# deepmarkpy/aware

Hardware: AMD Instinct MI355X
Metric: waveform-seconds/sec through embed->attack->detect; BER vs reference (higher is better)
Workload: dtype f32 accumulation on the 16-bit MFMA pipe; conv-block GEMMs: every f32 operand scaled by a power of two and carried as TWO binary16 terms (within one f32 ulp of the operand, rms 2^-24.5), 3 partial products, the l_a*l_b term (<= 2^-22) dropped -- gemm_h2.hip: error level of an f32 dot product (agains

## Files before the change

aware_amd/csrc/capi.hip:

```cpp
#include <hip/hip_runtime.h>
#include <math.h>
#include <stdio.h>
#include <stdlib.h>
#include <string.h>
#include <string>
#include <algorithm>
#include <vector>

#include "../../include/aware_hip.h"
#include "common.hpp"
#include "kernels.h"

using namespace aware;

static thread_local std::string g_last_err;

#define HIPCHK(expr)                                                                  \
    do {                                                                              \
        hipError_t _e = (expr);                                                       \
        if (_e != hipSuccess) {                                                       \
            g_last_err = std::string(#expr) + ": " + hipGetErrorString(_e);           \
            return AWARE_E_HIP;                                                       \
        }                                                                             \
    } while (0)
#define LAUNCHCHK() HIPCHK(hipGetLastError())

struct LaunchProfiler {
    hipStream_t st;
    std::vector<hipEvent_t> ev;
    std::vector<int> kind;
};
static thread_local LaunchProfiler* g_prof = nullptr;
static inline void prof_mark(int kind) {
    if (!g_prof) return;
    hipEvent_t e;
    if (hipEventCreate(&e) != hipSuccess) return;
    (void)hipEventRecord(e, g_prof->st);
    g_prof->ev.push_back(e);
    g_prof->kind.push_back(kind);
}
#define PROF(kind) prof_mark(kind)
enum { K_SYNTH = 0, K_ANALYSIS = 1, K_GEMM = 2, K_MELNORM = 3, K_INLRELU = 4, K_HEAD = 5, K_SYNTH_ADJ = 6,
       K_ANALYSIS_ADJ = 7, K_MISC = 8, K_GEMM_CLIP_FWD = 9, K_GEMM_CLIP_BWD = 10, K_GEMM_X3_FWD = 11, K_GEMM_X3_BWD = 12 };

static int absmax_into_scratch(const float* in, const int* off, const int* len, int B, int max_len, void* scratch,
                               unsigned long long** pmax_out, int** pcount_out, int* ps_out, hipStream_t st);

struct aware_plan {
    PlanDev dev;
    void* mem = nullptr;
};

struct aware_batch {
    int B = 0;
    std::vector<int> n, in_off, T, frame_off, pool_off, out_off, out_len, pc_in, pc_syn;
    int NF = 0, NP = 0, NS = 0, max_frames = 0, max_len = 0, pstride = 0;
    int uniform_tp = 0;
    int synth_run = kSynthBlocks;
    int* d_mem = nullptr;
    int *d_frame_off = nullptr, *d_pool_off = nullptr, *d_in_off = nullptr, *d_in_len = nullptr, *d_out_off = nullptr,
        *d_out_len = nullptr, *d_pc_in = nullptr, *d_pc_syn = nullptr;
    int an_run = 0, n_an_wg = 0, n_syn_wg = 0;
    int *d_an_wg = nullptr, *d_syn_wg = nullptr;
    std::vector<int> an_wg, syn_wg;
    int* d_order = nullptr;
    std::vector<int> order;
};

struct aware_detector {
    int n_mels = 0, n_layers = 0, nbits = 0;
    int band_lo = 0, nband = 0;
    int ch[8] = {0};
    int maxc = 0;
    float* mem = nullptr;
    float* melT = nullptr;
    float* melB = nullptr;
    float* w[8] = {nullptr};
    float* wT[8] = {nullptr};
    void* wpk[8] = {nullptr};
    void* wTpk[8] = {nullptr};
    void* melTpk = nullptr;
    void* melBpk = nullptr;
    void* lastpk = nullptr;
    void* lastTpk = nullptr;
    void* pkmem = nullptr;
    void* wh2[8] = {nullptr};
    void* wTh2[8] = {nullptr};
    void* h2mem = nullptr;
    float* bias[8] = {nullptr};
    void* mel2mem = nullptr;
    float2* melw = nullptr;
    unsigned char* melm = nullptr;
    float* melf_w = nullptr;
    unsigned char* melf_s = nullptr;
};

extern "C" int aware_version(void) { return 300; }
extern "C" const char* aware_last_hip_error(void) { return g_last_err.c_str(); }

extern "C" int aware_plan_create(aware_plan** out, int n_fft, int hop, int win_length, int window, int band_lo_bin,
                                 int band_hi_bin) {
    if (!out) return AWARE_E_BADARG;
    if (n_fft != kNfft || hop != kHop || win_length != kNfft) return AWARE_E_UNSUPPORTED;
    if (window != 0 && window != 1) return AWARE_E_BADARG;
    const int nband = band_hi_bin - band_lo_bin + 1;
    if (band_lo_bin < 1 || band_hi_bin > 511 || nband < 1 || nband > kFS) return AWARE_E_UNSUPPORTED;
    const double PI = 3.14159265358979323846;
    std::vector<float> h(2 * 512 + 2 * 512 + 1024 + 1024 + 3 * 768);
    float* tw512 = h.data();
    float* tw1024 = tw512 + 1024;
    float* win = tw1024 + 1024;
    float* win2 = win + 1024;
    for (int j = 0; j < 512; ++j) {
        tw512[2 * j] = (float)cos(2 * PI * j / 512);
        tw512[2 * j + 1] = (float)-sin(2 * PI * j / 512);
        tw1024[2 * j] = (float)cos(2 * PI * j / 1024);
        tw1024[2 * j + 1] = (float)-sin(2 * PI * j / 1024);
// ... 41 lines not shown
    b->B = B;
    b->n.assign(n_samples, n_samples + B);
    b->in_off.resize(B);
    b->T.resize(B);
    b->frame_off.resize(B + 1);
    b->pool_off.resize(B + 1);
    b->out_off.resize(B);
    b->out_len.resize(B);
    b->pc_in.resize(B);
    b->pc_syn.resize(B);
    int acc = 0, max_pc = 1;
    for (int rb : {12, 8, 6, 4}) {
        long runs = 0;
        for (int i = 0; i < B; ++i) runs += (n_samples[i] / kHop + rb - 1) / rb;
        bool ok = true;
        for (int i = 0; i < B && ok; ++i) {
            const int nb = n_samples[i] / kHop, ns = (nb + rb - 1) / rb;
            if (ns > 1 && nb / ns < 3) ok = false;
        }
        if (!ok) continue;
        b->synth_run = rb;
        if (runs >= 4096) break;
    }
    b->frame_off[0] = 0;
    b->pool_off[0] = 0;
    for (int i = 0; i < B; ++i) {
        const int n = n_samples[i];
        if (n <= kHalf) { delete b; return AWARE_E_BADARG; }
        b->in_off[i] = in_offsets ? in_offsets[i] : acc;
        acc += n;
        const int T = 1 + n / kHop;
        b->T[i] = T;
        b->frame_off[i + 1] = b->frame_off[i] + T;
        b->pool_off[i + 1] = b->pool_off[i] + ((T / 2 + 31) & ~31);
        b->out_off[i] = kHop * (b->frame_off[i] - i);
        b->out_len[i] = kHop * (T - 1);
        b->pc_in[i] = (n + 4095) / 4096;
        int nseg = (T - 1 + b->synth_run - 1) / b->synth_run;
        if (nseg < 1) nseg = 1;
        b->pc_syn[i] = nseg;
        if (T > b->max_frames) b->max_frames = T;
        if (n > b->max_len) b->max_len = n;
        if (b->pc_in[i] > max_pc) max_pc = b->pc_in[i];
        if (nseg > max_pc) max_pc = nseg;
    }
    b->NF = b->frame_off[B];
    b->NP = b->pool_off[B];
    b->uniform_tp = b->T[0] / 2;
    for (int i = 1; i < B; ++i)
        if (b->T[i] / 2 != b->uniform_tp) b->uniform_tp = 0;
    b->NS = kHop * (b->NF - B);
    b->pstride = max_pc;
    {
        constexpr int kAnalysisMaxRun = 12;
        auto total_runs = [&](int r) { long t = 0; for (int i = 0; i < B; ++i) t += (b->T[i] + r - 1) / r; return t; };
        int R = 4;
        for (int cand = kAnalysisMaxRun; cand >= 4; --cand)
            if (total_runs(cand) >= 4096) { R = cand; break; }
        bool same = true;
        for (int i = 1; i < B; ++i) same = same && b->T[i] == b->T[0];
        if (same)
            for (int cand = R; cand >= 4 && cand >= R - 3; --cand)
                if (((b->T[0] + cand - 1) / cand) % kStreamWaves == 0) { R = cand; break; }
        b->an_run = R;
        if (B < (1 << 19) && b->max_frames / 4 < 4096 * kStreamWaves) {
            for (int i = 0; i < B; ++i) {
                const int ra = (b->T[i] + R - 1) / R, rs = std::max(1, (b->T[i] - 1 + b->synth_run - 1) / b->synth_run);
                for (int w = 0; w < (ra + kStreamWaves - 1) / kStreamWaves; ++w) b->an_wg.push_back((i << 12) | w);
                for (int w = 0; w < (rs + kStreamWaves - 1) / kStreamWaves; ++w) b->syn_wg.push_back((i << 12) | w);
            }
        }
        b->n_an_wg = (int)b->an_wg.size();
        b->n_syn_wg = (int)b->syn_wg.size();
    }
    b->order.resize(B);
    for (int i = 0; i < B; ++i) b->order[i] = i;
    std::stable_sort(b->order.begin(), b->order.end(), [&](int x, int y) { return b->T[x] > b->T[y]; });
    const size_t ints = (size_t)(B + 1) * 2 + (size_t)B * 7 + b->an_wg.size() + b->syn_wg.size();
    HIPCHK(hipMalloc((void**)&b->d_mem, ints * sizeof(int)));
    int* d = b->d_mem;
    auto up = [&](int*& dst, const std::vector<int>& v) -> hipError_t {
        dst = d;
        d += v.size();
        return hipMemcpy(dst, v.data(), v.size() * sizeof(int), hipMemcpyHostToDevice);
    };
    HIPCHK(up(b->d_frame_off, b->frame_off));
    HIPCHK(up(b->d_pool_off, b->pool_off));
    HIPCHK(up(b->d_in_off, b->in_off));
    HIPCHK(up(b->d_in_len, b->n));
    HIPCHK(up(b->d_out_off, b->out_off));
    HIPCHK(up(b->d_out_len, b->out_len));
    HIPCHK(up(b->d_pc_in, b->pc_in));
    HIPCHK(up(b->d_pc_syn, b->pc_syn));
    HIPCHK(up(b->d_order, b->order));
    if (b->n_an_wg) HIPCHK(up(b->d_an_wg, b->an_wg));
    if (b->n_syn_wg) HIPCHK(up(b->d_syn_wg, b->syn_wg));
    *out = b;
    return AWARE_OK;
}
extern "C" void aware_batch_destroy(aware_batch* b) {
    if (!b) return;
    if (b->d_mem) (void)hipFree(b->d_mem);
    delete b;
}
extern "C" int aware_batch_total_frames(const aware_batch* b) { return b ? b->NF : AWARE_E_BADARG; }
extern "C" int aware_batch_total_pooled(const aware_batch* b) { return b ? b->NP : AWARE_E_BADARG; }
extern "C" int aware_batch_total_out(const aware_batch* b) { return b ? b->NS : AWARE_E_BADARG; }
extern "C" int aware_batch_out_offset(const aware_batch* b, int i) {
    return (b && i >= 0 && i < b->B) ? b->out_off[i] : AWARE_E_BADARG;
}
extern "C" int aware_batch_out_length(const aware_batch* b, int i) {
    return (b && i >= 0 && i < b->B) ? b->out_len[i] : AWARE_E_BADARG;
}
extern "C" int aware_batch_frames(const aware_batch* b, int i) {
    return (b && i >= 0 && i < b->B) ? b->T[i] : AWARE_E_BADARG;
}
extern "C" size_t aware_batch_scratch_bytes(const aware_batch* b) {
    return b ? (size_t)b->B * b->pstride * sizeof(unsigned long long) + 256 : 0;
}

static void run_analysis(AnalysisLaunch& L, int dsp_path, hipStream_t st) {
    if (dsp_path == 0 && !L.full && stream_supported(L.plan)) { L.stream = 1; launch_analysis_stream(L, st); }
    else launch_analysis(L, st);
}
static void run_synth(SynthLaunch& S, int dsp_path, hipStream_t st) {
    if (dsp_path == 0 && !S.full && stream_supported(S.plan)) { S.stream = 1; launch_synth_stream(S, st); }
    else launch_synth(S, st);
}

struct Carver {
    char* base;
    size_t off = 0, cap;
    bool ok = true;
    Carver(void* p, size_t c) : base((char*)p), cap(c) {}
    template <typename Tp> Tp* take(size_t count) {
        off = (off + 255) & ~(size_t)255;
        Tp* r = (Tp*)(base + off);
        off += count * sizeof(Tp);
        if (off > cap) ok = false;
        return r;
    }
};

extern "C" int aware_stft(const aware_plan* plan, const aware_batch* b, const float* audio, int normalize, void* spec,
                          void* scratch, void* stream) {
    if (!plan || !b || !audio || !spec || (normalize && !scratch)) return AWARE_E_BADARG;
    hipStream_t st = (hipStream_t)stream;
    unsigned long long* pmax = (unsigned long long*)scratch;
// ... 986 lines not shown
    HIPCHK(hipMemcpyAsync(e->target, target, (size_t)b->B * e->det->nbits * sizeof(float), hipMemcpyDeviceToDevice, st));
    HIPCHK(hipMemsetAsync(e->step, 0, 4 * sizeof(int), st));
    HIPCHK(hipMemsetD32Async((hipDeviceptr_t)e->best_loss, 0x7F800000, b->B, st));
    if (e->opt.active) {
        HIPCHK(hipMemcpyAsync(e->opt.d_lr, e->opt.lr_init.data(), (size_t)b->B * sizeof(double), hipMemcpyHostToDevice, st));
        HIPCHK(hipMemcpyAsync(e->opt.d_state, e->opt.state_init.data(), (size_t)b->B * 3 * sizeof(double), hipMemcpyHostToDevice, st));
    }
    e->steps_done = 0;
    return AWARE_OK;
}

static int embed_iteration(aware_embed* e, hipStream_t st, int do_step, float* grad_out) {
    const aware_batch* b = e->b;
    const aware_detector* d = e->det;
    SynthLaunch S;
    S.plan = e->plan->dev; S.frame_off = b->d_frame_off; S.B = b->B; S.max_frames = b->max_frames; S.run_blocks = b->synth_run; S.wg_tab = b->d_syn_wg; S.n_wg = b->n_syn_wg;
    S.amp = e->coef; S.ph = e->P; S.out = e->yraw; S.add = e->oob; S.pmax = e->pmaxY; S.pstride = b->pstride;
    S.c0 = e->pl1 ? e->c0 : nullptr; S.pl1 = e->pl1;
    const int dsp = e->cfg.dsp_path;
    run_synth(S, dsp, st);
    LAUNCHCHK(); PROF(K_SYNTH);
    if (e->pl1) {
        launch_l1_reduce(e->pl1, b->d_pc_syn, b->pstride, b->d_frame_off, e->plan->dev.nband, e->cfg.l1_weight, e->l1term, b->B, st);
        LAUNCHCHK(); PROF(K_MISC);
    }
    AnalysisLaunch L;
    L.plan = e->plan->dev; L.frame_off = b->d_frame_off; L.B = b->B; L.max_frames = b->max_frames; L.run_frames = b->an_run; L.wg_tab = b->d_an_wg; L.n_wg = b->n_an_wg;
    L.sig = e->yraw; L.sig_off = b->d_out_off; L.sig_len = b->d_out_len;
    L.pmax = e->pmaxY; L.pcount = b->d_pc_syn; L.pstride = b->pstride; L.double_norm = 1;
    L.mag = e->mag; L.unit = e->U; L.unit_default = 0.f; L.write_pad = 0;
    const bool mel_taps = dsp == 0 && d->melw && d->melm && stream_supported(e->plan->dev) && e->cfg.mel == 0;
    const bool mel_fold = mel_taps && d->melf_w && d->melf_s && d->n_mels == 128;
    if (mel_fold) { L.mel_out = e->db.xm; L.melf_w = d->melf_w; L.melf_s = d->melf_s; }
    run_analysis(L, dsp, st);
    LAUNCHCHK(); PROF(K_ANALYSIS);
    DetGradCtx G;
    G.pipe = e->cfg.conv_pipe; G.readout = e->cfg.readout; G.target = e->target; G.loss_kind = e->cfg.loss;
    G.loss = e->loss; G.d1 = e->d1; G.d2 = e->d2; G.gmag = e->gmag; G.loss_add = e->l1term;
    G.step = do_step ? e->step : nullptr;
    G.best_loss = do_step ? e->best_loss : nullptr;
    G.improved = do_step ? e->improved : nullptr;
    G.mel_grad_only = mel_taps;
    G.xm_ready = mel_fold;
    int rc = det_forward_backward(d, b, e->mag, e->db, G, st);
    if (rc) return rc;
    SynthLaunch SA;
    SA.plan = e->plan->dev; SA.frame_off = b->d_frame_off; SA.B = b->B; SA.max_frames = b->max_frames; SA.run_blocks = b->synth_run; SA.wg_tab = b->d_syn_wg; SA.n_wg = b->n_syn_wg;
    SA.amp = e->gmag; SA.ph = e->U; SA.out = e->gy; SA.adjoint = 1; SA.yraw = e->yraw; SA.pmax_in = e->pmaxY;
    SA.pcount = b->d_pc_syn; SA.pdot = e->pdot; SA.pstride = b->pstride; SA.gpad = e->gpad;
    if (mel_taps) { SA.dmel = e->db.xm; SA.melw = d->melw; SA.melm = d->melm; }
    run_synth(SA, dsp, st);
    LAUNCHCHK(); PROF(K_SYNTH_ADJ);
    AnalysisLaunch LA;
    LA.plan = e->plan->dev; LA.frame_off = b->d_frame_off; LA.B = b->B; LA.max_frames = b->max_frames; LA.run_frames = b->an_run; LA.wg_tab = b->d_an_wg; LA.n_wg = b->n_an_wg;
    LA.sig = e->gy; LA.sig_off = b->d_out_off; LA.sig_len = b->d_out_len;
    LA.pmax = e->pmaxY; LA.pcount = b->d_pc_syn; LA.pstride = b->pstride;
    LA.adjoint = 1; LA.yraw = e->yraw; LA.pdot = e->pdot; LA.phasor = e->P;
    LA.coef = e->coef; LA.mom = e->mom; LA.vel = e->vel; LA.lo = e->lo; LA.hi = e->hi; LA.best = e->best;
    LA.improved = e->improved; LA.sched = e->sched; LA.sched_len = e->cfg.num_iterations + 1; LA.step = e->step;
    const bool own_step = do_step && e->opt.active;
    LA.grad_out = own_step ? e->gmag : grad_out; LA.do_step = own_step ? 0 : do_step;
    memcpy(LA.hyp, e->hyp, sizeof(LA.hyp));
    LA.gpad = e->gpad; LA.c0 = e->c0; LA.box_ratio = (float)pow(10.0, -(double)e->cfg.tolerance_db / 20.0);
    LA.l1_weight = e->pl1 ? e->cfg.l1_weight : 0.f;
    run_analysis(LA, dsp, st);
    LAUNCHCHK(); PROF(K_ANALYSIS_ADJ);
    if (own_step) {
        const auto& o = e->opt;
        launch_opt_rows(o.kind, e->coef, e->gmag, e->mom, e->vel, e->c0, LA.box_ratio, e->best, e->improved, b->d_frame_off, b->B,
                        b->NF, o.d_tab, e->cfg.num_iterations, e->step, o.plateau ? o.d_lr : nullptr, o.wd, o.hyp,
                        e->plan->dev.nband, st);
        if (o.plateau)
            launch_plateau(e->loss, o.d_state, o.d_lr, b->B, o.factor, o.patience, o.threshold, o.min_lr, o.eps, st);
        LAUNCHCHK(); PROF(K_MISC);
    }
    return AWARE_OK;
}

extern "C" int aware_embed_iterate(aware_embed* e, int n_iters, void* stream) {
    if (!e || n_iters < 0) return AWARE_E_BADARG;
    if (e->steps_done + n_iters > e->cfg.num_iterations) return AWARE_E_BADARG;
    hipStream_t st = (hipStream_t)stream;
    if (!e->cfg.use_graph) {
        for (int i = 0; i < n_iters; ++i) {
            int rc = embed_iteration(e, st, 1, nullptr);
            if (rc) return rc;
            ++e->steps_done;
        }
        return AWARE_OK;
    }
    constexpr int kGraphIters = 16;
    if (!e->gexec) {
        if (!e->cap) HIPCHK(hipStreamCreateWithFlags(&e->cap, hipStreamNonBlocking));
        for (int which = 0; which < 2; ++which) {
            HIPCHK(hipStreamBeginCapture(e->cap, hipStreamCaptureModeThreadLocal));
            int rc = AWARE_OK;
            for (int i = 0; i < (which ? kGraphIters : 1) && rc == AWARE_OK; ++i) rc = embed_iteration(e, e->cap, 1, nullptr);
            hipGraph_t g = nullptr;
            hipError_t ce = hipStreamEndCapture(e->cap, &g);
            hipGraphExec_t ge = nullptr;
            if (rc == AWARE_OK && ce == hipSuccess) ce = hipGraphInstantiate(&ge, g, nullptr, nullptr, 0);
            if (rc != AWARE_OK || ce != hipSuccess) {
                if (ge) (void)hipGraphExecDestroy(ge);
                if (g) (void)hipGraphDestroy(g);
                if (e->gexec) { (void)hipGraphExecDestroy(e->gexec); e->gexec = nullptr; }
                if (e->graph) { (void)hipGraphDestroy(e->graph); e->graph = nullptr; }
                if (rc != AWARE_OK) return rc;
// ... 254 lines not shown
```

aware_amd/csrc/dsp_stream.hip:

```cpp
#include "common.hpp"
#include "dsp_args.hpp"
#include "kernels.h"

namespace aware {

constexpr int kSW = kStreamWaves;
constexpr int kSThreads = 64 * kSW;

__device__ __forceinline__ ClipNorm clip_norm_wave(const unsigned long long* part, int nseg, int lane) {
    unsigned long long v = 0;
    for (int i = lane; i < nseg; i += 64) v = umax64(v, part[i]);
    v = wave_max64(v);
    ClipNorm c;
    const float raw = __uint_as_float((unsigned)(v >> 32));
    c.k = 0xFFFFFFFFu - (unsigned)(v & 0xFFFFFFFFu);
    c.m = raw + 1e-8f;
    c.m2 = raw / c.m + 1e-8f;
    return c;
}
__device__ __forceinline__ double dot_wave(const double* part, int nseg, int lane) {
    double s = 0.0;
    for (int i = lane; i < nseg; i += 64) s += part[i];
    return wave_sum_d(s);
}

struct LaneEnv {
    float2 lo, hi;
};
__device__ __forceinline__ LaneEnv lane_env(const PlanDev& pl, int lane) {
    LaneEnv e;
    e.lo = make_float2(fast_rcp(pl.env_tab[768 + 2 * lane]), fast_rcp(pl.env_tab[768 + 2 * lane + 1]));
    e.hi = make_float2(fast_rcp(pl.env_tab[768 + 128 + 2 * lane]), fast_rcp(pl.env_tab[768 + 128 + 2 * lane + 1]));
    return e;
}
__device__ __forceinline__ float env_at(const PlanDev& pl, int p, int T) {
    return T < 4 ? ola_envelope_loop(pl.window2, p, T) : pl.env_tab[ola_envelope_index(p, T)];
}

template <int MODE, bool L1, bool MELF = false>
__global__ __launch_bounds__(kSThreads, MODE == AN_ADJ ? 3 : 4) void analysis_stream_kernel(AnalysisArgs a, int run_frames) {
    __shared__ float magrow_s[MELF ? kSW : 1][MELF ? kFS : 1];
    __shared__ cf tw1s[512];
    __shared__ cf tw2s[64];
    __shared__ float2 wins[512];
    __shared__ cf scratch[kSW][kFftScratch];
    const int tid = threadIdx.x;
    fft_fill_tables(tid, kSThreads, a.plan.tw512, tw1s, tw2s);
    for (int i = tid; i < 512; i += kSThreads) wins[i] = make_float2(a.plan.window[2 * i], a.plan.window[2 * i + 1]);
    __syncthreads();

    int b = blockIdx.y, wgx = blockIdx.x;
    if (a.wg_tab) { const int e = a.wg_tab[blockIdx.x]; b = e >> 12; wgx = e & 4095; }
    const int f0 = a.frame_off[b];
    const int T = a.frame_off[b + 1] - f0;
    const int wave = __builtin_amdgcn_readfirstlane(tid >> 6), lane = tid & 63;
    const int t0 = (wgx * kSW + wave) * run_frames;
    if (t0 >= T) return;
    const int nfr = min(run_frames, T - t0);
    const int n = a.sig_len[b];
    const float* x = a.sig + a.sig_off[b];
    const bool al8 = (reinterpret_cast<uintptr_t>(x) & 7) == 0;

    float m = 1.f, m2 = 1.f;
    unsigned kmax = 0xFFFFFFFFu;
    if (a.pmax) {
        const ClipNorm cn = clip_norm_wave(a.pmax + (size_t)b * a.pstride, a.pcount[b], lane);
        m = cn.m;
        m2 = (MODE == AN_ADJ || a.double_norm) ? cn.m2 : 1.f;
        kmax = cn.k;
    }
    const float inv_m = 1.0f / m, inv_m2 = 1.0f / m2, inv_mm2 = 1.0f / (m * m2);
    float corr = 0.f;
    const float* gpL = nullptr;
    const float* gpR = nullptr;
    LaneEnv le;
    le.lo = le.hi = make_float2(1.f, 1.f);
    if (MODE == AN_ADJ) {
        const float adot = (float)dot_wave(a.pdot + (size_t)b * a.pstride, a.pcount[b], lane);
        const float yk = a.yraw[a.sig_off[b] + kmax];
        corr = adot * ((yk > 0.f) ? 1.f : ((yk < 0.f) ? -1.f : 0.f));
        gpL = a.gpad + (size_t)b * 1024;
        gpR = gpL + 512;
        le = lane_env(a.plan, lane);
    }

    auto load_half = [&](int P) -> float2 {
        const int s_lo = P - kHalf;
        float2 v;
        if (MODE == AN_NORM) {
            if (al8 && s_lo >= 0 && s_lo + 128 <= n) {
                v = *reinterpret_cast<const float2*>(x + s_lo + 2 * lane);
            } else {
                int s0 = s_lo + 2 * lane, s1 = s0 + 1;
                s0 = s0 < 0 ? -s0 : s0;
                s1 = s1 < 0 ? -s1 : s1;
                s0 = s0 >= n ? 2 * (n - 1) - s0 : s0;
                s1 = s1 >= n ? 2 * (n - 1) - s1 : s1;
                v.x = x[min(max(s0, 0), n - 1)];
                v.y = x[min(max(s1, 0), n - 1)];
            }
            if (a.pmax) {
                v.x = v.x * inv_m;
                v.y = v.y * inv_m;
                if (a.double_norm) { v.x = v.x * inv_m2; v.y = v.y * inv_m2; }
            }
            return v;
        }
        if (al8 && T >= 4 && s_lo >= 513 && s_lo + 127 <= n - 514 && P >= 768 && P + 127 < kHop * T) {
            float2 g = *reinterpret_cast<const float2*>(x + s_lo + 2 * lane);
            const unsigned s = (unsigned)(s_lo + 2 * lane);
            if (s == kmax) g.x -= corr;
            if (s + 1 == kmax) g.y -= corr;
            g.x = g.x * inv_mm2;
            g.y = g.y * inv_mm2;
            const float2 re = (P & 128) ? le.hi : le.lo;
            return make_float2(g.x * re.x, g.y * re.y);
        }
        float o[2];
#pragma unroll
        for (int e = 0; e < 2; ++e) {
            const int p = P + 2 * lane + e;
            const int src = p - kHalf;
            const bool valid = src >= 0 && src < n;
            float g = x[min(max(src, 0), n - 1)];
            const bool cl = src >= 1 && src <= kHalf;
            const bool cr = src >= n - kHalf - 1 && src <= n - 2;
            const float pl = gpL[min(max(kHalf - src, 0), 511)];
            const float pr = gpR[min(max(n - 2 - src, 0), 511)];
            if (cl) g += pl;
            if (cr) g += pr;
            if ((unsigned)src == kmax) g -= corr;
            g = g * inv_mm2;
            o[e] = valid ? g * fast_rcp(env_at(a.plan, p, T)) : 0.f;
        }
        return make_float2(o[0], o[1]);
    };

    cf* s = scratch[wave];
    const int band_lo = a.plan.band_lo, nband = a.plan.nband;
    cf w1024[5];
#pragma unroll
    for (int r = 0; r < 5; ++r) w1024[r] = a.plan.tw1024[lane + 64 * r];
    float4 sc = make_float4(0.f, 0.f, 1.f, 0.f);
    float inv_bc2 = 1.f;
    int improved = 0;
    if (MODE == AN_ADJ && a.do_step) {
        sc = a.sched[min(max(*a.step - 1, 0), a.sched_len - 1)];
        inv_bc2 = 1.0f / sc.z;
        improved = a.improved[b];
    }

    const float l1g = (MODE == AN_ADJ && L1) ? a.l1_weight / (float)(nband * T) : 0.f;
    float wA[kMelTapsA], wB[kMelTapsB];
    int sA = 0, sB = 0;
    if (MELF) {
#pragma unroll
        for (int j = 0; j < kMelTapsA; ++j) wA[j] = a.melf_w[(size_t)lane * kMelTapsB + j];
#pragma unroll
        for (int j = 0; j < kMelTapsB; ++j) wB[j] = a.melf_w[(size_t)(lane + 64) * kMelTapsB + j];
        sA = a.melf_s[lane];
        sB = a.melf_s[lane + 64];
#pragma unroll
        for (int r = 0; r < 8; ++r) {
            const int f = lane + 64 * r - band_lo;
            if (f >= nband && f < kFS) magrow_s[MELF ? wave : 0][f] = 0.f;
        }
    }
    float2 raw[8];
#pragma unroll
    for (int r = 0; r < 8; ++r) raw[r] = load_half(kHop * t0 + 128 * r);

#pragma unroll 1
    for (int fr = 0; fr < nfr; ++fr) {
        const int t = t0 + fr;
        const size_t row = (size_t)(f0 + t);
        cf preP[5];
        float preM[5], preV[5], preC[5], pre0[5];
        if (MODE == AN_ADJ) {
#pragma unroll
            for (int r = 0; r < 5; ++r) {
                const int f = lane + 64 * r - band_lo;
                const size_t idx = row * kFS + (size_t)min(max(f, 0), kFS - 1);
                preP[r] = a.phasor[idx];
                if (a.do_step) { preM[r] = a.mom[idx]; preV[r] = a.vel[idx]; preC[r] = a.coef[idx]; }
                else { preM[r] = preV[r] = 0.f; preC[r] = L1 ? a.coef[idx] : 0.f; }
                pre0[r] = (a.do_step || L1) ? a.c0[idx] : 0.f;
            }
        }
        cf v[8];
#pragma unroll
        for (int r = 0; r < 8; ++r) {
            const float2 w = wins[lane + 64 * r];
            v[r] = mk(raw[r].x * w.x, raw[r].y * w.y);
        }
#pragma unroll
        for (int r = 0; r < 6; ++r) raw[r] = raw[r + 2];
        raw[6] = load_half(kHop * (t + 1) + 768);
        raw[7] = load_half(kHop * (t + 1) + 896);
        fft512_wave_t<-1>(lane, v, tw1s, tw2s, s);

        const int src_lane = (64 - lane) & 63;
#pragma unroll
        for (int r = 0; r < 5; ++r) {
            cf zp = mk(__shfl(v[7 - r].x, src_lane), __shfl(v[7 - r].y, src_lane));
            if (lane == 0) zp = (r == 0) ? v[0] : v[8 - r];
            const int k = lane + 64 * r;
            const int f = k - band_lo;
            if (f < 0 || f >= nband) continue;
            const cf zk = v[r];
            const cf e = mk(0.5f * (zk.x + zp.x), 0.5f * (zk.y - zp.y));
            const cf d = mk(0.5f * (zk.x - zp.x), 0.5f * (zk.y + zp.y));
            const cf wd = cmul(w1024[r], d);
            const cf X = mk(e.x + wd.y, e.y - wd.x);
            const size_t idx = row * kFS + f;
            if (MODE == AN_NORM) {
                const float mg = fast_sqrt(X.x * X.x + X.y * X.y);
                const float im = fast_rcp(mg);
                if (MELF) magrow_s[wave][f] = mg;
                else if (a.mag) a.mag[idx] = mg;
                if (a.unit) a.unit[idx] = (mg > 0.f) ? mk(X.x * im, X.y * im) : mk(a.unit_default, 0.f);
            } else {
                const cf P = preP[r];
                float g = (X.x * P.x + X.y * P.y) * (1.0f / 512.0f);
                if (L1) {
                    const float dc = preC[r] - pre0[r];
                    g += l1g * ((dc > 0.f) ? 1.f : ((dc < 0.f) ? -1.f : 0.f));
                }
                if (a.grad_out) a.grad_out[idx] = g;
                if (a.do_step) {
                    float mo = preM[r], ve = preV[r], p = preC[r];
                    float blo, bhi;
                    box_bounds(pre0[r], a.box_ratio, blo, bhi);
                    nadam_clamp_update(p, mo, ve, g, blo, bhi, sc.x, sc.y, inv_bc2, a.hyp);
                    a.mom[idx] = mo; a.vel[idx] = ve; a.coef[idx] = p;
                    if (improved) a.best[idx] = p;
                }
            }
        }
        if (MODE == AN_NORM && MELF) {
            float* mr = magrow_s[MELF ? wave : 0];
            float m0 = 0.f, m1 = 0.f;
#pragma unroll
            for (int j = 0; j < kMelTapsA; ++j) m0 += wA[j] * mr[sA + j];
#pragma unroll
            for (int j = 0; j < kMelTapsB; ++j) m1 += wB[j] * mr[sB + j];
            float* mo = a.mel_out + row * 128;
            mo[lane] = m0;
            mo[lane + 64] = m1;
        }
        if (MODE == AN_NORM && a.write_pad) {
#pragma unroll
            for (int r = 0; r < 8; ++r) {
                const int f = lane + 64 * r - band_lo;
                if (f >= nband && f < kFS) {
                    const size_t idx = row * kFS + f;
                    if (a.mag) a.mag[idx] = 0.f;
                    if (a.unit) a.unit[idx] = mk(0.f, 0.f);
                }
            }
        }
    }
}

template <int MODE, bool L1, bool MELG = false>
__global__ __launch_bounds__(kSThreads, 4) void synth_stream_kernel(SynthArgs a) {
    __shared__ float2 melw_s[MELG ? kFS : 1];
    __shared__ float melrow_s[MELG ? kSW : 1][MELG ? 128 : 1];
    __shared__ cf tw1s[512];
    __shared__ cf tw2s[64];
    __shared__ float2 wins[512];
    __shared__ cf mcs[512];
    __shared__ cf scratch[kSW][kFftScratch];
    const int tid = threadIdx.x;
    const float scale = (MODE == SY_FWD) ? (1.0f / 512.0f) : 1.0f;
    fft_fill_tables(tid, kSThreads, a.plan.tw512, tw1s, tw2s);
    for (int i = tid; i < 512; i += kSThreads) {
        wins[i] = make_float2(a.plan.window[2 * i] * scale, a.plan.window[2 * i + 1] * scale);
        const cf w = a.plan.tw1024[i];
        mcs[i] = (i < 256) ? mk(0.5f * (1.f + w.y), 0.5f * w.x) : mk(0.5f * (1.f - w.y), -0.5f * w.x);
    }
    if (MELG)
        for (int i = tid; i < kFS; i += kSThreads) melw_s[i] = a.melw[i];
    __syncthreads();

    int b = blockIdx.y, wgx = blockIdx.x;
    if (a.wg_tab) { const int e = a.wg_tab[blockIdx.x]; b = e >> 12; wgx = e & 4095; }
    const int f0 = a.frame_off[b];
    const int T = a.frame_off[b + 1] - f0;
    const int nblk = T - 1;
    const int wave = __builtin_amdgcn_readfirstlane(tid >> 6), lane = tid & 63;
    const int run = wgx * kSW + wave;
    int nseg, jb0, jb1;
    synth_segment(nblk, run, a.run_blocks, nseg, jb0, jb1);
    if (run >= nseg || T < 1) return;
    const bool first = jb0 == 0, last = jb1 == nblk;
    const int t_lo = max(jb0 - 1, 0);
    const int t_hi = (MODE == SY_ADJ && last) ? T + 2 : jb1 + 1;
    const int Ny = kHop * nblk;
    const int so = sig_offset(a.frame_off, b);
    float* out = a.out + so;
    const float* add = (MODE == SY_FWD && a.add) ? a.add + so : nullptr;
    const float* y = (MODE == SY_ADJ) ? a.yraw + so : nullptr;
    float inv_m = 1.f, inv_m2 = 1.f;
    if (MODE == SY_ADJ) {
        const ClipNorm cn = clip_norm_wave(a.pmax_in + (size_t)b * a.pstride, a.pcount[b], lane);
        inv_m = 1.0f / cn.m;
        inv_m2 = 1.0f / cn.m2;
    }
    const LaneEnv le = lane_env(a.plan, lane);
    const int band_lo = a.plan.band_lo, nband = a.plan.nband;
    cf* s = scratch[wave];

    float inA[8];
    cf inP[8];
    unsigned fo[8];
    unsigned inband = 0;
#pragma unroll
    for (int r = 0; r < 8; ++r) {
        const int k = lane + 64 * r;
        const int f = ((k <= 256) ? k : 512 - k) - band_lo;
        fo[r] = (unsigned)min(max(f, 0), kFS - 1);
        if (f >= 0 && f < nband) inband |= 1u << r;
    }
    unsigned mtap[2] = {0u, 0u};
    float drow[2] = {0.f, 0.f};
    if (MELG) {
#pragma unroll
        for (int r = 0; r < 8; ++r) mtap[r >> 2] |= (unsigned)a.melm[fo[r]] << (8 * (r & 3));
    }
    auto load_band = [&](int t) {
        const size_t row = (size_t)(f0 + t);
        const float* A = MELG ? nullptr : a.amp + row * kFS;
        const cf* P = a.ph + row * kFS;
        if (MELG) {
            const float* D = a.dmel + row * 128;
            drow[0] = D[lane];
            drow[1] = D[lane + 64];
        }
#pragma unroll
        for (int r = 0; r < 8; ++r) {
            inP[r] = P[fo[r]];
            if (!MELG) {
                const float am = A[fo[r]];
                inA[r] = ((inband >> r) & 1u) ? am : 0.f;
            }
        }
    };
    auto expand_mel = [&]() {
        float* mr = melrow_s[MELG ? wave : 0];
        mr[lane] = drow[0];
        mr[lane + 64] = drow[1];
#pragma unroll
        for (int r = 0; r < 8; ++r) {
            const unsigned m = (mtap[r >> 2] >> (8 * (r & 3))) & 0xFFu;
            const float2 w = melw_s[MELG ? fo[r] : 0];
            const float v = w.x * mr[m] + w.y * mr[m + 1];
            inA[r] = ((inband >> r) & 1u) ? v : 0.f;
            if (r == 3) __builtin_amdgcn_sched_barrier(0);
        }
    };

    float2 acc[6];
#pragma unroll
    for (int q = 0; q < 6; ++q) acc[q] = make_float2(0.f, 0.f);
    unsigned long long best = 0;
    double dot = 0.0;
    float l1 = 0.f;
    if (t_lo <= T - 1) load_band(t_lo);

    auto epi_operands = [&](int i, bool emit, float2& e0, float2& e1) {
        e0 = make_float2(0.f, 0.f);
        e1 = e0;
        if (emit) {
            const float* src = (MODE == SY_FWD) ? add : y;
            if (src) {
                e0 = *reinterpret_cast<const float2*>(src + kHop * i + 2 * lane);
                e1 = *reinterpret_cast<const float2*>(src + kHop * i + 128 + 2 * lane);
            }
        }
    };
    auto ola_emit = [&](int i, bool emit, const float2 (&c)[8], const float2 e0, const float2 e1) {
        const float2 o0 = make_float2(acc[0].x + c[0].x, acc[0].y + c[0].y);
        const float2 o1 = make_float2(acc[1].x + c[1].x, acc[1].y + c[1].y);
#pragma unroll
        for (int q = 0; q < 4; ++q) acc[q] = make_float2(acc[q + 2].x + c[q + 2].x, acc[q + 2].y + c[q + 2].y);
        acc[4] = c[6];
        acc[5] = c[7];

        const int j0 = kHop * i + 2 * lane, j1 = j0 + 128;
        if (MODE == SY_FWD) {
            if (emit) {
                float2 r0, r1;
                if (T >= 4 && i >= 1 && i <= T - 3) { r0 = le.lo; r1 = le.hi; }
                else {
                    r0 = make_float2(fast_rcp(env_at(a.plan, kHalf + j0, T)), fast_rcp(env_at(a.plan, kHalf + j0 + 1, T)));
                    r1 = make_float2(fast_rcp(env_at(a.plan, kHalf + j1, T)), fast_rcp(env_at(a.plan, kHalf + j1 + 1, T)));
                }
                float2 v0 = make_float2(o0.x * r0.x, o0.y * r0.y), v1 = make_float2(o1.x * r1.x, o1.y * r1.y);
                if (add) { v0.x += e0.x; v0.y += e0.y; v1.x += e1.x; v1.y += e1.y; }
                *reinterpret_cast<float2*>(out + j0) = v0;
                *reinterpret_cast<float2*>(out + j1) = v1;
                best = umax64(best, pack_max(fabsf(v0.x), (unsigned)j0));
                best = umax64(best, pack_max(fabsf(v0.y), (unsigned)j0 + 1));
                best = umax64(best, pack_max(fabsf(v1.x), (unsigned)j1));
                best = umax64(best, pack_max(fabsf(v1.y), (unsigned)j1 + 1));
            }
        } else {
            if (emit) {
                *reinterpret_cast<float2*>(out + j0) = o0;
                *reinterpret_cast<float2*>(out + j1) = o1;
                dot += (double)o0.x * (double)((e0.x * inv_m) * inv_m2) + (double)o0.y * (double)((e0.y * inv_m) * inv_m2);
                dot += (double)o1.x * (double)((e1.x * inv_m) * inv_m2) + (double)o1.y * (double)((e1.y * inv_m) * inv_m2);
            } else if (first && i < 0 && i >= -2) {
                float* gp = a.gpad + (size_t)b * 1024;
                const int p0 = kHop * (i + 2) + 2 * lane, p1 = p0 + 128;
                *reinterpret_cast<float2*>(gp + p0) = o0;
                *reinterpret_cast<float2*>(gp + p1) = o1;
                const float ov[4] = {o0.x, o0.y, o1.x, o1.y};
                const int pp[4] = {p0, p0 + 1, p1, p1 + 1};
#pragma unroll
                for (int e = 0; e < 4; ++e) {
                    const int j = kHalf - pp[e];
                    const float yv = y[min(max(j, 0), max(Ny - 1, 0))];
                    if (j >= 1 && j < Ny) dot += (double)ov[e] * (double)((yv * inv_m) * inv_m2);
                }
            } else if (last && i >= nblk && i <= nblk + 1) {
                float* gp = a.gpad + (size_t)b * 1024 + 512;
                const int u0 = kHop * (i - nblk) + 2 * lane, u1 = u0 + 128;
                *reinterpret_cast<float2*>(gp + u0) = o0;
                *reinterpret_cast<float2*>(gp + u1) = o1;
                const float ov[4] = {o0.x, o0.y, o1.x, o1.y};
                const int uu[4] = {u0, u0 + 1, u1, u1 + 1};
#pragma unroll
                for (int e = 0; e < 4; ++e) {
                    const int j = Ny - 2 - uu[e];
                    const float yv = y[min(max(j, 0), max(Ny - 1, 0))];
                    if (j >= 0) dot += (double)ov[e] * (double)((yv * inv_m) * inv_m2);
                }
            }
        }
    };

    const int t_fft = min(t_hi, T - 1);
#pragma unroll 1
    for (int t = t_lo; t <= t_fft; ++t) {
        const int i = t - 2;
        const bool emit = i >= jb0 && i < jb1;
        float2 e0, e1;
        epi_operands(i, emit, e0, e1);
        float2 c[8];
        {
            if (MELG) expand_mel();
            if (MODE == SY_FWD && L1 && ((t >= jb0 && t < jb1) || (last && t == T - 1))) {
                const float* C0 = a.c0 + (size_t)(f0 + t) * kFS;
#pragma unroll
                for (int r = 0; r < 5; ++r) {
                    const int f = lane + 64 * r - band_lo;
                    const float cv = C0[min(max(f, 0), kFS - 1)];
                    if (f >= 0 && f < nband && (r < 4 || lane == 0)) l1 += fabsf(inA[r] - cv);
                }
            }
            cf v[8];
#pragma unroll
            for (int r = 0; r < 8; ++r) {
                const cf mc = mcs[lane + 64 * r];
                const float xr = inA[r] * inP[r].x, xi = (r < 4) ? inA[r] * inP[r].y : -(inA[r] * inP[r].y);
                v[r] = mk(xr * mc.x - xi * mc.y, xr * mc.y + xi * mc.x);
            }
            load_band(min(t + 1, T - 1));
            fft512_wave_t<1>(lane, v, tw1s, tw2s, s);
#pragma unroll
            for (int r = 0; r < 8; ++r) {
                const float2 w = wins[lane + 64 * r];
                c[r] = make_float2(v[r].x * w.x, v[r].y * w.y);
            }
        }
        ola_emit(i, emit, c, e0, e1);
    }
#pragma unroll 1
    for (int t = t_fft + 1; t <= t_hi; ++t) {
        const int i = t - 2;
        const bool emit = i >= jb0 && i < jb1;
        float2 e0, e1;
        epi_operands(i, emit, e0, e1);
        float2 c[8];
#pragma unroll
        for (int r = 0; r < 8; ++r) c[r] = make_float2(0.f, 0.f);
        ola_emit(i, emit, c, e0, e1);
    }
    if (MODE == SY_FWD) {
        if (a.pmax) {
            best = wave_max64(best);
            if (lane == 0) a.pmax[(size_t)b * a.pstride + run] = best;
        }
        if (L1) {
            const double tot = wave_sum_d((double)l1);
            if (lane == 0) a.pl1[(size_t)b * a.pstride + run] = tot;
        }
    } else {
        dot = wave_sum_d(dot);
        if (lane == 0) a.pdot[(size_t)b * a.pstride + run] = dot;
    }
}

__global__ __launch_bounds__(64) void l1_reduce_kernel(const double* __restrict__ pl1, const int* __restrict__ pcount, int pstride,
                                                        const int* __restrict__ frame_off, int nband, float weight,
                                                        float* __restrict__ l1term) {
    const int b = blockIdx.x, lane = threadIdx.x;
    const double s = dot_wave(pl1 + (size_t)b * pstride, pcount[b], lane);
    const int T = frame_off[b + 1] - frame_off[b];
    if (lane == 0) l1term[b] = weight * (float)(s / (double)(nband * T));
}
void launch_l1_reduce(const double* pl1, const int* pcount, int pstride, const int* frame_off, int nband, float weight,
                      float* l1term, int B, hipStream_t st) {
    hipLaunchKernelGGL(l1_reduce_kernel, dim3(B), dim3(64), 0, st, pl1, pcount, pstride, frame_off, nband, weight, l1term);
}

bool stream_supported(const PlanDev& plan) { return plan.band_lo >= 1 && plan.band_lo + plan.nband <= 257; }

void launch_analysis_stream(const AnalysisLaunch& L, hipStream_t st) {
    AnalysisArgs a{};
    a.plan = L.plan;
    a.frame_off = L.frame_off;
    a.sig = L.sig; a.sig_off = L.sig_off; a.sig_len = L.sig_len;
    a.pmax = L.pmax; a.pcount = L.pcount; a.pstride = L.pstride;
    a.double_norm = L.double_norm; a.unit_default = L.unit_default;
    a.mag = L.mag; a.unit = (cf*)L.unit; a.full = nullptr;
    a.yraw = L.yraw; a.pdot = L.pdot; a.phasor = (const cf*)L.phasor;
    a.coef = L.coef; a.mom = L.mom; a.vel = L.vel; a.lo = L.lo; a.hi = L.hi; a.best = L.best;
    a.improved = L.improved; a.sched = (const float4*)L.sched; a.sched_len = L.sched_len > 0 ? L.sched_len : 1; a.step = L.step;
    a.grad_out = L.grad_out; a.do_step = L.do_step;
    a.hyp = make_float4(L.hyp[0], L.hyp[1], L.hyp[2], L.hyp[3]);
    a.gpad = L.gpad; a.write_pad = L.write_pad;
    a.c0 = L.c0; a.box_ratio = L.box_ratio; a.l1_weight = L.l1_weight;
    int R = 4;
    dim3 grid;
    if (L.run_frames >= 4 && L.run_frames <= 16 && L.wg_tab && L.n_wg > 0) {
        R = L.run_frames;
        a.wg_tab = L.wg_tab;
        grid = dim3((unsigned)L.n_wg, 1, 1);
    } else {
        for (int cand = 16; cand >= 4; --cand)
            if ((long)L.B * ((L.max_frames + cand - 1) / cand) >= 4096) { R = cand; break; }
        for (int cand = R; cand >= 4 && cand >= R - 3; --cand)
            if (((L.max_frames + cand - 1) / cand) % kSW == 0) { R = cand; break; }
        const int runs = (L.max_frames + R - 1) / R;
        grid = dim3((unsigned)((runs + kSW - 1) / kSW), (unsigned)L.B, 1);
    }
    if (L.adjoint && a.l1_weight != 0.f) hipLaunchKernelGGL((analysis_stream_kernel<AN_ADJ, true>), grid, dim3(kSThreads), 0, st, a, R);
    else if (L.adjoint) hipLaunchKernelGGL((analysis_stream_kernel<AN_ADJ, false>), grid, dim3(kSThreads), 0, st, a, R);
    else if (L.mel_out && L.melf_w && L.melf_s) {
        a.mel_out = L.mel_out; a.melf_w = L.melf_w; a.melf_s = L.melf_s; a.mag = nullptr;
        hipLaunchKernelGGL((analysis_stream_kernel<AN_NORM, false, true>), grid, dim3(kSThreads), 0, st, a, R);
    } else hipLaunchKernelGGL((analysis_stream_kernel<AN_NORM, false>), grid, dim3(kSThreads), 0, st, a, R);
}

void launch_synth_stream(const SynthLaunch& L, hipStream_t st) {
    SynthArgs a{};
    a.plan = L.plan;
    a.frame_off = L.frame_off;
    a.amp = L.amp; a.ph = (const cf*)L.ph; a.full = nullptr;
    a.out = L.out; a.add = L.add; a.pmax = L.pmax; a.pstride = L.pstride;
    a.yraw = L.yraw; a.pmax_in = L.pmax_in; a.pcount = L.pcount; a.pdot = L.pdot; a.gpad = L.gpad;
    a.c0 = L.c0; a.pl1 = (L.c0 && L.pl1) ? L.pl1 : nullptr;
    const int nblk = L.max_frames - 1;
    a.run_blocks = (L.run_blocks >= 1 && L.run_blocks <= kSynthBlocks) ? L.run_blocks : kSynthBlocks;
    int runs = (nblk + a.run_blocks - 1) / a.run_blocks;
    if (runs < 1) runs = 1;
    dim3 grid((unsigned)((runs + kSW - 1) / kSW), (unsigned)L.B, 1);
    if (L.wg_tab && L.n_wg > 0 && a.run_blocks == L.run_blocks) {
        a.wg_tab = L.wg_tab;
        grid = dim3((unsigned)L.n_wg, 1, 1);
    }
    a.dmel = L.dmel; a.melw = (const float2*)L.melw; a.melm = L.melm;
    if (L.adjoint && L.dmel && L.melw && L.melm) hipLaunchKernelGGL((synth_stream_kernel<SY_ADJ, false, true>), grid, dim3(kSThreads), 0, st, a);
    else if (L.adjoint) hipLaunchKernelGGL((synth_stream_kernel<SY_ADJ, false>), grid, dim3(kSThreads), 0, st, a);
    else if (a.pl1) hipLaunchKernelGGL((synth_stream_kernel<SY_FWD, true>), grid, dim3(kSThreads), 0, st, a);
    else hipLaunchKernelGGL((synth_stream_kernel<SY_FWD, false>), grid, dim3(kSThreads), 0, st, a);
}

}
```

aware_amd/csrc/kernels.h:

```cpp
#pragma once
#include <hip/hip_runtime.h>
#include <stddef.h>
#include <stdint.h>
#include "common.hpp"

namespace aware {

constexpr int kStreamWaves = 4;

struct AnalysisLaunch {
    PlanDev plan;
    const int* frame_off = nullptr;
    int B = 0, max_frames = 0;
    int run_frames = 0, n_wg = 0;
    const int* wg_tab = nullptr;
    const float* sig = nullptr;
    const int* sig_off = nullptr;
    const int* sig_len = nullptr;
    const unsigned long long* pmax = nullptr;
    const int* pcount = nullptr;
    int pstride = 0;
    int double_norm = 0;
    float unit_default = 0.f;
    float* mag = nullptr;
    void* unit = nullptr;
    void* full = nullptr;
    int adjoint = 0;
    const float* yraw = nullptr;
    const double* pdot = nullptr;
    const void* phasor = nullptr;
    float* coef = nullptr; float* mom = nullptr; float* vel = nullptr;
    const float* lo = nullptr; const float* hi = nullptr; float* best = nullptr;
    const int* improved = nullptr;
    const void* sched = nullptr;
    int sched_len = 0;
    const int* step = nullptr;
    float* grad_out = nullptr;
    int do_step = 0;
    float hyp[4] = {0.1f, 0.999f, 0.001f, 1e-8f};
    int stream = 0;
    const float* gpad = nullptr;
    int write_pad = 1;
    const float* c0 = nullptr;
    float box_ratio = 0.f;
    float l1_weight = 0.f;
    float* mel_out = nullptr;
    const float* melf_w = nullptr;
    const unsigned char* melf_s = nullptr;
};
struct SynthLaunch {
    PlanDev plan;
    const int* frame_off = nullptr;
    int B = 0, max_frames = 0;
    int n_wg = 0;
    const int* wg_tab = nullptr;
    const float* amp = nullptr;
    const void* ph = nullptr;
    const void* full = nullptr;
    float* out = nullptr;
    const float* add = nullptr;
    unsigned long long* pmax = nullptr;
// ... 141 lines not shown
```

Baseline: 1926.

## Tune adjoint analysis run length and cut per-lane register state in stream kernels

Adds a separate run-length and workgroup table for the adjoint analysis pass, chosen with its own max run and wave target instead of reusing the forward analysis settings. In the analysis kernel, the 1024-point twiddles move from per-lane registers into LDS, and per-frame epilogue operands (phasor, moments, coef, c0) are software-prefetched one frame ahead. In the synthesis kernel, per-lane band slot indices, in-band masks and reciprocal envelope values move into shared tables. The aim is lower register pressure, better occupancy and hidden global-load latency, at the cost of more LDS use and extra prefetch registers.

```diff
diff --git a/aware_amd/csrc/capi.hip b/aware_amd/csrc/capi.hip
--- a/aware_amd/csrc/capi.hip
+++ b/aware_amd/csrc/capi.hip
@@ -60,9 +60,9 @@
     int* d_mem = nullptr;
     int *d_frame_off = nullptr, *d_pool_off = nullptr, *d_in_off = nullptr, *d_in_len = nullptr, *d_out_off = nullptr,
         *d_out_len = nullptr, *d_pc_in = nullptr, *d_pc_syn = nullptr;
-    int an_run = 0, n_an_wg = 0, n_syn_wg = 0;
-    int *d_an_wg = nullptr, *d_syn_wg = nullptr;
-    std::vector<int> an_wg, syn_wg;
+    int an_run = 0, adj_run = 0, n_an_wg = 0, n_adj_wg = 0, n_syn_wg = 0;
+    int *d_an_wg = nullptr, *d_adj_wg = nullptr, *d_syn_wg = nullptr;
+    std::vector<int> an_wg, adj_wg, syn_wg;
     int* d_order = nullptr;
     std::vector<int> order;
 };
@@ -210,31 +210,37 @@
     b->NS = kHop * (b->NF - B);
     b->pstride = max_pc;
     {
-        constexpr int kAnalysisMaxRun = 12;
         auto total_runs = [&](int r) { long t = 0; for (int i = 0; i < B; ++i) t += (b->T[i] + r - 1) / r; return t; };
-        int R = 4;
-        for (int cand = kAnalysisMaxRun; cand >= 4; --cand)
-            if (total_runs(cand) >= 4096) { R = cand; break; }
         bool same = true;
         for (int i = 1; i < B; ++i) same = same && b->T[i] == b->T[0];
-        if (same)
-            for (int cand = R; cand >= 4 && cand >= R - 3; --cand)
-                if (((b->T[0] + cand - 1) / cand) % kStreamWaves == 0) { R = cand; break; }
-        b->an_run = R;
+        auto pick_run = [&](int max_run, long waves) {
+            int R = 4;
+            for (int cand = max_run; cand >= 4; --cand)
+                if (total_runs(cand) >= waves) { R = cand; break; }
+            if (same)
+                for (int cand = R; cand >= 4 && cand >= R - 3; --cand)
+                    if (((b->T[0] + cand - 1) / cand) % kStreamWaves == 0) { R = cand; break; }
+            return R;
+        };
+        b->an_run = pick_run(kAnalysisMaxRun, kAnalysisWaves);
+        b->adj_run = pick_run(kAdjointMaxRun, kAdjointWaves);
         if (B < (1 << 19) && b->max_frames / 4 < 4096 * kStreamWaves) {
             for (int i = 0; i < B; ++i) {
-                const int ra = (b->T[i] + R - 1) / R, rs = std::max(1, (b->T[i] - 1 + b->synth_run - 1) / b->synth_run);
+                const int ra = (b->T[i] + b->an_run - 1) / b->an_run, rj = (b->T[i] + b->adj_run - 1) / b->adj_run;
+                const int rs = std::max(1, (b->T[i] - 1 + b->synth_run - 1) / b->synth_run);
                 for (int w = 0; w < (ra + kStreamWaves - 1) / kStreamWaves; ++w) b->an_wg.push_back((i << 12) | w);
+                for (int w = 0; w < (rj + kStreamWaves - 1) / kStreamWaves; ++w) b->adj_wg.push_back((i << 12) | w);
                 for (int w = 0; w < (rs + kStreamWaves - 1) / kStreamWaves; ++w) b->syn_wg.push_back((i << 12) | w);
             }
         }
         b->n_an_wg = (int)b->an_wg.size();
+        b->n_adj_wg = (int)b->adj_wg.size();
         b->n_syn_wg = (int)b->syn_wg.size();
     }
     b->order.resize(B);
     for (int i = 0; i < B; ++i) b->order[i] = i;
     std::stable_sort(b->order.begin(), b->order.end(), [&](int x, int y) { return b->T[x] > b->T[y]; });
-    const size_t ints = (size_t)(B + 1) * 2 + (size_t)B * 7 + b->an_wg.size() + b->syn_wg.size();
+    const size_t ints = (size_t)(B + 1) * 2 + (size_t)B * 7 + b->an_wg.size() + b->adj_wg.size() + b->syn_wg.size();
     HIPCHK(hipMalloc((void**)&b->d_mem, ints * sizeof(int)));
     int* d = b->d_mem;
     auto up = [&](int*& dst, const std::vector<int>& v) -> hipError_t {
@@ -252,6 +258,7 @@
     HIPCHK(up(b->d_pc_syn, b->pc_syn));
     HIPCHK(up(b->d_order, b->order));
     if (b->n_an_wg) HIPCHK(up(b->d_an_wg, b->an_wg));
+    if (b->n_adj_wg) HIPCHK(up(b->d_adj_wg, b->adj_wg));
     if (b->n_syn_wg) HIPCHK(up(b->d_syn_wg, b->syn_wg));
     *out = b;
     return AWARE_OK;
@@ -1344,7 +1351,7 @@
     run_synth(SA, dsp, st);
     LAUNCHCHK(); PROF(K_SYNTH_ADJ);
     AnalysisLaunch LA;
-    LA.plan = e->plan->dev; LA.frame_off = b->d_frame_off; LA.B = b->B; LA.max_frames = b->max_frames; LA.run_frames = b->an_run; LA.wg_tab = b->d_an_wg; LA.n_wg = b->n_an_wg;
+    LA.plan = e->plan->dev; LA.frame_off = b->d_frame_off; LA.B = b->B; LA.max_frames = b->max_frames; LA.run_frames = b->adj_run; LA.wg_tab = b->d_adj_wg; LA.n_wg = b->n_adj_wg;
     LA.sig = e->gy; LA.sig_off = b->d_out_off; LA.sig_len = b->d_out_len;
     LA.pmax = e->pmaxY; LA.pcount = b->d_pc_syn; LA.pstride = b->pstride;
     LA.adjoint = 1; LA.yraw = e->yraw; LA.pdot = e->pdot; LA.phasor = e->P;
diff --git a/aware_amd/csrc/dsp_stream.hip b/aware_amd/csrc/dsp_stream.hip
--- a/aware_amd/csrc/dsp_stream.hip
+++ b/aware_amd/csrc/dsp_stream.hip
@@ -43,10 +43,12 @@
     __shared__ cf tw1s[512];
     __shared__ cf tw2s[64];
     __shared__ float2 wins[512];
+    __shared__ cf w1ks[320];
     __shared__ cf scratch[kSW][kFftScratch];
     const int tid = threadIdx.x;
     fft_fill_tables(tid, kSThreads, a.plan.tw512, tw1s, tw2s);
     for (int i = tid; i < 512; i += kSThreads) wins[i] = make_float2(a.plan.window[2 * i], a.plan.window[2 * i + 1]);
+    for (int i = tid; i < 320; i += kSThreads) w1ks[i] = a.plan.tw1024[i];
     __syncthreads();
 
     int b = blockIdx.y, wgx = blockIdx.x;
@@ -138,9 +140,6 @@
 
     cf* s = scratch[wave];
     const int band_lo = a.plan.band_lo, nband = a.plan.nband;
-    cf w1024[5];
-#pragma unroll
-    for (int r = 0; r < 5; ++r) w1024[r] = a.plan.tw1024[lane + 64 * r];
     float4 sc = make_float4(0.f, 0.f, 1.f, 0.f);
     float inv_bc2 = 1.f;
     int improved = 0;
@@ -170,23 +169,33 @@
 #pragma unroll
     for (int r = 0; r < 8; ++r) raw[r] = load_half(kHop * t0 + 128 * r);
 
+    struct EpiOps {
+        cf P[5];
+        float M[5], V[5], C[5], Z[5];
+    };
+    auto load_ops = [&](int t) -> EpiOps {
+        EpiOps o;
+        const size_t row = (size_t)(f0 + t);
+#pragma unroll
+        for (int r = 0; r < 5; ++r) {
+            const int f = lane + 64 * r - band_lo;
+            const size_t idx = row * kFS + (size_t)min(max(f, 0), kFS - 1);
+            o.P[r] = a.phasor[idx];
+            o.M[r] = a.do_step ? a.mom[idx] : 0.f;
+            o.V[r] = a.do_step ? a.vel[idx] : 0.f;
+            o.C[r] = (a.do_step || L1) ? a.coef[idx] : 0.f;
+            o.Z[r] = (a.do_step || L1) ? a.c0[idx] : 0.f;
+        }
+        return o;
+    };
+    EpiOps cur{}, nxt{};
+    if (MODE == AN_ADJ) cur = load_ops(t0);
+
 #pragma unroll 1
     for (int fr = 0; fr < nfr; ++fr) {
         const int t = t0 + fr;
         const size_t row = (size_t)(f0 + t);
-        cf preP[5];
-        float preM[5], preV[5], preC[5], pre0[5];
-        if (MODE == AN_ADJ) {
-#pragma unroll
-            for (int r = 0; r < 5; ++r) {
-                const int f = lane + 64 * r - band_lo;
-                const size_t idx = row * kFS + (size_t)min(max(f, 0), kFS - 1);
-                preP[r] = a.phasor[idx];
-                if (a.do_step) { preM[r] = a.mom[idx]; preV[r] = a.vel[idx]; preC[r] = a.coef[idx]; }
-                else { preM[r] = preV[r] = 0.f; preC[r] = L1 ? a.coef[idx] : 0.f; }
-                pre0[r] = (a.do_step || L1) ? a.c0[idx] : 0.f;
-            }
-        }
+        if (MODE == AN_ADJ) nxt = load_ops(t0 + min(fr + 1, nfr - 1));
         cf v[8];
 #pragma unroll
         for (int r = 0; r < 8; ++r) {
@@ -210,7 +219,7 @@
             const cf zk = v[r];
             const cf e = mk(0.5f * (zk.x + zp.x), 0.5f * (zk.y - zp.y));
             const cf d = mk(0.5f * (zk.x - zp.x), 0.5f * (zk.y + zp.y));
-            const cf wd = cmul(w1024[r], d);
+            const cf wd = cmul(w1ks[lane + 64 * r], d);
             const cf X = mk(e.x + wd.y, e.y - wd.x);
             const size_t idx = row * kFS + f;
             if (MODE == AN_NORM) {
@@ -220,23 +229,24 @@
                 else if (a.mag) a.mag[idx] = mg;
                 if (a.unit) a.unit[idx] = (mg > 0.f) ? mk(X.x * im, X.y * im) : mk(a.unit_default, 0.f);
             } else {
-                const cf P = preP[r];
+                const cf P = cur.P[r];
                 float g = (X.x * P.x + X.y * P.y) * (1.0f / 512.0f);
                 if (L1) {
-                    const float dc = preC[r] - pre0[r];
+                    const float dc = cur.C[r] - cur.Z[r];
                     g += l1g * ((dc > 0.f) ? 1.f : ((dc < 0.f) ? -1.f : 0.f));
                 }
                 if (a.grad_out) a.grad_out[idx] = g;
                 if (a.do_step) {
-                    float mo = preM[r], ve = preV[r], p = preC[r];
+                    float mo = cur.M[r], ve = cur.V[r], p = cur.C[r];
                     float blo, bhi;
-                    box_bounds(pre0[r], a.box_ratio, blo, bhi);
+                    box_bounds(cur.Z[r], a.box_ratio, blo, bhi);
                     nadam_clamp_update(p, mo, ve, g, blo, bhi, sc.x, sc.y, inv_bc2, a.hyp);
                     a.mom[idx] = mo; a.vel[idx] = ve; a.coef[idx] = p;
                     if (improved) a.best[idx] = p;
                 }
             }
         }
+        if (MODE == AN_ADJ) cur = nxt;
         if (MODE == AN_NORM && MELF) {
             float* mr = magrow_s[MELF ? wave : 0];
             float m0 = 0.f, m1 = 0.f;
@@ -270,6 +280,8 @@
     __shared__ cf tw2s[64];
     __shared__ float2 wins[512];
     __shared__ cf mcs[512];
+    __shared__ unsigned slot_s[512];
+    __shared__ float2 renv_s[128];
     __shared__ cf scratch[kSW][kFftScratch];
     const int tid = threadIdx.x;
     const float scale = (MODE == SY_FWD) ? (1.0f / 512.0f) : 1.0f;
@@ -279,6 +291,12 @@
         const cf w = a.plan.tw1024[i];
         mcs[i] = (i < 256) ? mk(0.5f * (1.f + w.y), 0.5f * w.x) : mk(0.5f * (1.f - w.y), -0.5f * w.x);
     }
+    for (int i = tid; i < 512; i += kSThreads) {
+        const int f = ((i <= 256) ? i : 512 - i) - a.plan.band_lo;
+        slot_s[i] = (unsigned)min(max(f, 0), kFS - 1) | ((f >= 0 && f < a.plan.nband) ? 1u << 16 : 0u);
+    }
+    for (int i = tid; i < 128; i += kSThreads)
+        renv_s[i] = make_float2(fast_rcp(a.plan.env_tab[768 + 2 * i]), fast_rcp(a.plan.env_tab[768 + 2 * i + 1]));
     if (MELG)
         for (int i = tid; i < kFS; i += kSThreads) melw_s[i] = a.melw[i];
     __syncthreads();
@@ -307,26 +325,18 @@
         inv_m = 1.0f / cn.m;
         inv_m2 = 1.0f / cn.m2;
     }
-    const LaneEnv le = lane_env(a.plan, lane);
     const int band_lo = a.plan.band_lo, nband = a.plan.nband;
     cf* s = scratch[wave];
 
     float inA[8];
     cf inP[8];
-    unsigned fo[8];
-    unsigned inband = 0;
-#pragma unroll
-    for (int r = 0; r < 8; ++r) {
-        const int k = lane + 64 * r;
-        const int f = ((k <= 256) ? k : 512 - k) - band_lo;
-        fo[r] = (unsigned)min(max(f, 0), kFS - 1);
-        if (f >= 0 && f < nband) inband |= 1u << r;
-    }
+    auto slot_col = [&](int r) -> unsigned { return slot_s[lane + 64 * r] & 0xFFFFu; };
+    auto slot_in = [&](int r) -> bool { return (slot_s[lane + 64 * r] >> 16) != 0u; };
     unsigned mtap[2] = {0u, 0u};
     float drow[2] = {0.f, 0.f};
     if (MELG) {
 #pragma unroll
-        for (int r = 0; r < 8; ++r) mtap[r >> 2] |= (unsigned)a.melm[fo[r]] << (8 * (r & 3));
+        for (int r = 0; r < 8; ++r) mtap[r >> 2] |= (unsigned)a.melm[slot_col(r)] << (8 * (r & 3));
     }
     auto load_band = [&](int t) {
         const size_t row = (size_t)(f0 + t);
@@ -339,10 +349,10 @@
         }
 #pragma unroll
         for (int r = 0; r < 8; ++r) {
-            inP[r] = P[fo[r]];
+            inP[r] = P[slot_col(r)];
             if (!MELG) {
-                const float am = A[fo[r]];
-                inA[r] = ((inband >> r) & 1u) ? am : 0.f;
+                const float am = A[slot_col(r)];
+                inA[r] = slot_in(r) ? am : 0.f;
             }
         }
     };
@@ -353,9 +363,9 @@
 #pragma unroll
         for (int r = 0; r < 8; ++r) {
             const unsigned m = (mtap[r >> 2] >> (8 * (r & 3))) & 0xFFu;
-            const float2 w = melw_s[MELG ? fo[r] : 0];
+            const float2 w = melw_s[MELG ? slot_col(r) : 0];
             const float v = w.x * mr[m] + w.y * mr[m + 1];
-            inA[r] = ((inband >> r) & 1u) ? v : 0.f;
+            inA[r] = slot_in(r) ? v : 0.f;
             if (r == 3) __builtin_amdgcn_sched_barrier(0);
         }
     };
@@ -391,7 +401,7 @@
         if (MODE == SY_FWD) {
             if (emit) {
                 float2 r0, r1;
-                if (T >= 4 && i >= 1 && i <= T - 3) { r0 = le.lo; r1 = le.hi; }
+                if (T >= 4 && i >= 1 && i <= T - 3) { r0 = renv_s[lane]; r1 = renv_s[64 + lane]; }
                 else {
                     r0 = make_float2(fast_rcp(env_at(a.plan, kHalf + j0, T)), fast_rcp(env_at(a.plan, kHalf + j0 + 1, T)));
                     r1 = make_float2(fast_rcp(env_at(a.plan, kHalf + j1, T)), fast_rcp(env_at(a.plan, kHalf + j1 + 1, T)));
@@ -455,9 +465,8 @@
                 const float* C0 = a.c0 + (size_t)(f0 + t) * kFS;
 #pragma unroll
                 for (int r = 0; r < 5; ++r) {
-                    const int f = lane + 64 * r - band_lo;
-                    const float cv = C0[min(max(f, 0), kFS - 1)];
-                    if (f >= 0 && f < nband && (r < 4 || lane == 0)) l1 += fabsf(inA[r] - cv);
+                    const float cv = C0[slot_col(r)];
+                    if (slot_in(r) && (r < 4 || lane == 0)) l1 += fabsf(inA[r] - cv);
                 }
             }
             cf v[8];
@@ -540,8 +549,10 @@
         a.wg_tab = L.wg_tab;
         grid = dim3((unsigned)L.n_wg, 1, 1);
     } else {
-        for (int cand = 16; cand >= 4; --cand)
-            if ((long)L.B * ((L.max_frames + cand - 1) / cand) >= 4096) { R = cand; break; }
+        const int max_run = L.adjoint ? kAdjointMaxRun : 16;
+        const long waves = L.adjoint ? kAdjointWaves : kAnalysisWaves;
+        for (int cand = max_run; cand >= 4; --cand)
+            if ((long)L.B * ((L.max_frames + cand - 1) / cand) >= waves) { R = cand; break; }
         for (int cand = R; cand >= 4 && cand >= R - 3; --cand)
             if (((L.max_frames + cand - 1) / cand) % kSW == 0) { R = cand; break; }
         const int runs = (L.max_frames + R - 1) / R;
diff --git a/aware_amd/csrc/kernels.h b/aware_amd/csrc/kernels.h
--- a/aware_amd/csrc/kernels.h
+++ b/aware_amd/csrc/kernels.h
@@ -7,6 +7,8 @@
 namespace aware {
 
 constexpr int kStreamWaves = 4;
+constexpr int kAnalysisMaxRun = 12, kAnalysisWaves = 4096;
+constexpr int kAdjointMaxRun = 16, kAdjointWaves = 3072;
 
 struct AnalysisLaunch {
     PlanDev plan;
```

After: 1933 (median of 6 runs). Within noise of the previous version (+0.4%).
